# MegviiRobot/CamLaserCalibraTool

Measured on NVIDIA H100. Metric: residual+Jacobian evals/sec (full LM solves), higher is better.
Workload: dtype f64

## Files before the change

camlasercalibratool_b200/_build.py:

```python
from __future__ import annotations

import os
import shutil
import subprocess

PKG_DIR = os.path.dirname(os.path.abspath(__file__))
CSRC = os.path.join(PKG_DIR, "csrc")
LIB_PATH = os.path.join(PKG_DIR, "libclc_b200.so")
SOURCES = ["clc_api.cu", "clc_pack.cpp"]
HEADERS = ["clc_kernels.cuh", "clc_math.cuh", "clc_lm.cuh", "clc_expand.cuh", "clc_linefit.cuh", "clc_camera.cuh", "clc_upload.inl"]
NVCC_FLAGS = [
    "-gencode", "arch=compute_90a,code=sm_90a",
    "-O3", "-lineinfo", "-std=c++17",
    "-shared", "-Xcompiler", "-fPIC",
    "-diag-suppress", "177",
]


def _nvcc() -> str:
    for cand in (shutil.which("nvcc"), "/usr/local/cuda/bin/nvcc"):
        if cand and os.path.exists(cand):
            return cand
    raise RuntimeError("nvcc not found: libclc_b200.so cannot be built")


def is_stale() -> bool:
    if not os.path.exists(LIB_PATH):
        return True
    t = os.path.getmtime(LIB_PATH)
    deps = [os.path.join(CSRC, f) for f in SOURCES + HEADERS]
    deps.append(os.path.join(PKG_DIR, "..", "include", "clc_b200.h"))
    return any(os.path.getmtime(d) > t for d in deps)


def build(force: bool = False, verbose: bool = False) -> str:
    if not force and not is_stale():
        return LIB_PATH
    extra = os.environ.get("CLC_NVCC_EXTRA", "").split()
    out = os.environ.get("CLC_LIB_OUT", LIB_PATH)
    cmd = [_nvcc(), *NVCC_FLAGS, *extra, "-o", out, *[os.path.join(CSRC, s) for s in SOURCES], "-ldl"]
    if verbose:
        cmd.insert(1, "-Xptxas")
        cmd.insert(2, "-v")
    res = subprocess.run(cmd, capture_output=True, text=True)
    if res.returncode != 0:
        raise RuntimeError("nvcc failed:\n" + res.stdout + res.stderr)
    if verbose:
        print(res.stderr)
    return out


REPO = os.path.dirname(PKG_DIR)
DROPIN_SRC = os.path.join(PKG_DIR, "host", "LaseCamCalB200.cpp")
BENCH_SRC = os.path.join(PKG_DIR, "host", "dropin_bench.cpp")
BENCH_EXE = os.path.join(PKG_DIR, "host", "clc_dropin_bench")
def interface_include_dirs():
    return [os.path.join(REPO, "tests", "stubs"), os.path.join(REPO, "include")]


def cxx_command(sources, out, extra=()):
    cxx = "/usr/bin/g++" if os.path.exists("/usr/bin/g++") else "g++"
    cmd = [cxx, "-O2", "-std=c++11", "-Wall"]
    for d in interface_include_dirs():
# ... 19 lines not shown
```

camlasercalibratool_b200/csrc/clc_api.cu:

```cuda
#include <cuda_runtime.h>
#include <dlfcn.h>
#include <nccl.h>

#include <algorithm>
#include <atomic>
#include <chrono>
#include <cstdio>
#include <cstdlib>
#include <cstring>
#include <mutex>
#include <string>
#include <vector>

#include "../../include/clc_b200.h"
#include "clc_kernels.cuh"
#include "clc_linefit.cuh"
#include "clc_small.cuh"

namespace {

thread_local std::string g_last_error;
std::atomic<int64_t> g_launches{0};

int fail(int code, const std::string& msg) {
  g_last_error = msg;
  return code;
}

#define CLC_CUDA(expr)                                                                                   \
  do {                                                                                                   \
    cudaError_t _e = (expr);                                                                             \
    if (_e != cudaSuccess)                                                                               \
      return fail(CLC_ERR_CUDA, std::string(#expr) + ": " + cudaGetErrorString(_e) + " (" __FILE__ ":" + \
                                    std::to_string(__LINE__) + ")");                                     \
  } while (0)

#define CLC_LAUNCH_CHECK()                  \
  do {                                      \
    g_launches.fetch_add(1);                \
    CLC_CUDA(cudaGetLastError());           \
  } while (0)

struct NcclApi {
  void* handle = nullptr;
  ncclResult_t (*GetUniqueId)(ncclUniqueId*) = nullptr;
  ncclResult_t (*CommInitRank)(ncclComm_t*, int, ncclUniqueId, int) = nullptr;
  ncclResult_t (*AllReduce)(const void*, void*, size_t, ncclDataType_t, ncclRedOp_t, ncclComm_t, cudaStream_t) = nullptr;
  ncclResult_t (*CommDestroy)(ncclComm_t) = nullptr;
  const char* (*GetErrorString)(ncclResult_t) = nullptr;
  std::string error;
};

NcclApi* nccl_api() {
  static NcclApi api;
  static bool tried = false;
  if (tried) return &api;
  tried = true;
  const char* names[] = {"libnccl.so.2", "libnccl.so"};
  for (const char* n : names) {
    api.handle = dlopen(n, RTLD_NOW | RTLD_GLOBAL);
    if (api.handle) break;
  }
  if (!api.handle) {
    api.error = std::string("dlopen(libnccl.so.2) failed: ") + dlerror();
    return &api;
  }
  api.GetUniqueId = reinterpret_cast<decltype(api.GetUniqueId)>(dlsym(api.handle, "ncclGetUniqueId"));
  api.CommInitRank = reinterpret_cast<decltype(api.CommInitRank)>(dlsym(api.handle, "ncclCommInitRank"));
// ... 102 lines not shown
  }
  for (int i = 0; i < n; ++i) x[perm[i]] = y[i];
}

int64_t round_up(int64_t v, int64_t m) { return (v + m - 1) / m * m; }

}

struct PinnedBlock {
  clc::LmState lm;
  double sums[clc::kMaxOut];
  double pose[8];
  int done;
  int nonplanar;
};
namespace {
std::mutex g_pinned_mutex;
std::vector<PinnedBlock*> g_pinned_free;
PinnedBlock* pinned_acquire() {
  {
    std::lock_guard<std::mutex> lock(g_pinned_mutex);
    if (!g_pinned_free.empty()) {
      PinnedBlock* b = g_pinned_free.back();
      g_pinned_free.pop_back();
      return b;
    }
  }
  PinnedBlock* b = nullptr;
  if (cudaMallocHost(&b, sizeof(PinnedBlock)) != cudaSuccess) return nullptr;
  return b;
}
void pinned_release(PinnedBlock* b) {
  if (!b) return;
  std::lock_guard<std::mutex> lock(g_pinned_mutex);
  g_pinned_free.push_back(b);
}
}

struct clc_comm {
  ncclComm_t comm = nullptr;
  int nranks = 1, rank = 0, device = 0;
  void* p2p_block = nullptr;
  void* peer_block[clc::kMaxRanks] = {};
  bool p2p_ready = false;
  bool local = false;
  size_t mailbox_bytes() const { return sizeof(unsigned long long) * 2 * 2 * (size_t)nranks * clc::kMailboxSlot; }
  size_t block_bytes() const { return mailbox_bytes() + sizeof(unsigned long long); }
};

struct clc_problem {
  int device = 0;
  cudaStream_t stream = nullptr;
  int num_sms = 0;
  int grid = 0;
  int64_t n_frames = 0, n_points = 0, n_points_padded = 0, n_edges = 0;
  int use_loss = 1;
  double cauchy_a = 0.05;
  double *x = nullptr, *y = nullptr, *z = nullptr;
  void *xy_block = nullptr, *z_block = nullptr;
  double* frame_pose = nullptr;
  double* frame_pose_true = nullptr;
  double* plane = nullptr;
  int64_t* offsets = nullptr;
  int* warp_first_frame = nullptr;
  double* edge_plane = nullptr;
  double* edge_pt = nullptr;
  unsigned long long* partials_ll = nullptr;
  unsigned int* launch_seq = nullptr;
  unsigned long long* pose_ll = nullptr;
  double* sums = nullptr;
  double* pose = nullptr;
  clc::LmState* lm = nullptr;
  double* flush_buf = nullptr;
  int64_t flush_n = 0;
  unsigned long long* timing = nullptr;
  bool use_pdl = true;
  int64_t l2_persist_bytes = 0;
  bool l2_window_set = false;
  bool small_kernel = true;
  int loop_in_kernel = 1;
  PinnedBlock* pinned = nullptr;
  double* h_sums = nullptr;
  int* h_done = nullptr;
  clc::LmState* h_lm = nullptr;
  clc_comm* comm_obj = nullptr;
  ncclComm_t comm = nullptr;
  int nranks = 1, rank = 0;
  int* p2p_error = nullptr;
  int allreduce_mode = 0;
  int64_t per_warp = 0;
  int grid_full = 0;
  cudaEvent_t ev0 = nullptr, ev1 = nullptr;
  int* d_nonplanar = nullptr;
  bool z_all_zero = false;
  bool host_planarity_known = false;
  bool planar = false;
  int planar_mode = 1;
  int64_t planar_min_points = 0;
};

namespace {

clc::ProblemView make_view(const clc_problem* p) {
  clc::ProblemView v;
  v.x = p->x; v.y = p->y; v.z = p->z;
  v.plane = p->plane;
  v.offsets = p->offsets;
  v.warp_first_frame = p->warp_first_frame;
  v.edge_plane = p->edge_plane;
  v.edge_pt = p->edge_pt;
  v.n_frames = p->n_frames;
  v.n_points = p->n_points;
  v.n_edges = p->n_edges;
  v.per_warp = p->per_warp;
  v.a2 = p->cauchy_a * p->cauchy_a;
  v.inv_a2 = 1.0 / v.a2;
  return v;
}

int set_device(const clc_problem* p) {
  CLC_CUDA(cudaSetDevice(p->device));
  return CLC_OK;
}

int launch_sweep(clc_problem* p, int mode, bool loss, bool edges, const double* d_pose, const int* d_done,
                 clc::LmState* d_lm, bool collective = true, bool pdl = false, int loop_sweeps = 1) {
  clc::SweepArgs a;
  a.pose7 = d_pose;
  a.done = d_done;
  a.partials_ll = p->partials_ll;
  a.sums = p->sums;
  a.launch_seq = p->launch_seq;
  a.pose_ll = p->pose_ll;
  a.lm = d_lm;
  a.use_loss = loss ? 1 : 0;
  a.use_edges = edges ? 1 : 0;
  a.loop_sweeps = loop_sweeps;
  a.timing = p->timing;
  a.nranks = 1;
  a.rank = 0;
  a.seq_counter = nullptr;
  a.error = p->p2p_error;
  if (p->nranks > 1 && p->allreduce_mode == 1 && collective) {
    clc_comm* c = p->comm_obj;
    a.nranks = c->nranks;
    a.rank = c->rank;
    a.seq_counter = reinterpret_cast<unsigned long long*>(static_cast<char*>(c->p2p_block) + c->mailbox_bytes());
    for (int r = 0; r < c->nranks; ++r) a.peer_mailbox[r] = static_cast<unsigned long long*>(c->peer_block[r]);
  }
  const clc::ProblemView v = make_view(p);
  cudaLaunchConfig_t cfg = {};
  cfg.gridDim = dim3((unsigned)p->grid);
  cfg.blockDim = dim3(clc::kThreads);
  cfg.dynamicSmemBytes = clc::dyn_smem_bytes(p->planar);
  cfg.stream = p->stream;
  cudaLaunchAttribute attr[1];
  attr[0].id = cudaLaunchAttributeProgrammaticStreamSerialization;
  attr[0].val.programmaticStreamSerializationAllowed = pdl ? 1 : 0;
  cfg.attrs = attr;
  cfg.numAttrs = 1;
  cudaError_t le;
  if (!p->planar && p->z == nullptr) return fail(CLC_ERR_INVALID, "internal: general sweep without a z stream");
  if (mode == clc::kModeClosedForm) {
    le = p->planar ? cudaLaunchKernelEx(&cfg, clc::clc_sweep_kernel<false, clc::kModeClosedForm, true>, v, a)
                   : cudaLaunchKernelEx(&cfg, clc::clc_sweep_kernel<false, clc::kModeClosedForm, false>, v, a);
  } else if (loop_sweeps > 1) {
    if (d_lm == nullptr) return fail(CLC_ERR_INVALID, "internal: looping sweep without an LM state");
    if (loss)
      le = p->planar ? cudaLaunchKernelEx(&cfg, clc::clc_sweep_kernel<true, clc::kModeLM, true, true>, v, a)
                     : cudaLaunchKernelEx(&cfg, clc::clc_sweep_kernel<true, clc::kModeLM, false, true>, v, a);
    else
      le = p->planar ? cudaLaunchKernelEx(&cfg, clc::clc_sweep_kernel<false, clc::kModeLM, true, true>, v, a)
                     : cudaLaunchKernelEx(&cfg, clc::clc_sweep_kernel<false, clc::kModeLM, false, true>, v, a);
  } else if (loss) {
    le = p->planar ? cudaLaunchKernelEx(&cfg, clc::clc_sweep_kernel<true, clc::kModeLM, true>, v, a)
                   : cudaLaunchKernelEx(&cfg, clc::clc_sweep_kernel<true, clc::kModeLM, false>, v, a);
  } else {
    le = p->planar ? cudaLaunchKernelEx(&cfg, clc::clc_sweep_kernel<false, clc::kModeLM, true>, v, a)
                   : cudaLaunchKernelEx(&cfg, clc::clc_sweep_kernel<false, clc::kModeLM, false>, v, a);
  }
  if (le != cudaSuccess) return fail(CLC_ERR_CUDA, std::string("sweep launch: ") + cudaGetErrorString(le));
  CLC_LAUNCH_CHECK();
  return CLC_OK;
}

int allreduce_sums(clc_problem* p, int count) {
  if (p->nranks <= 1 || p->allreduce_mode == 1) return CLC_OK;
  CLC_NCCL(nccl_api()->AllReduce(p->sums, p->sums, (size_t)count, ncclDouble, ncclSum, p->comm, p->stream));
  return CLC_OK;
}

cudaError_t sync_stream_low_latency(cudaStream_t st) {
  const auto t0 = std::chrono::steady_clock::now();
  for (;;) {
    const cudaError_t e = cudaStreamQuery(st);
    if (e != cudaErrorNotReady) return e;
    if (std::chrono::steady_clock::now() - t0 > std::chrono::microseconds(400)) return cudaStreamSynchronize(st);
#if defined(__x86_64__) || defined(__i386__)
    __builtin_ia32_pause();
#endif
  }
}

int check_p2p_error(clc_problem* p) {
  if (p->grid <= 1 && p->nranks <= 1) return CLC_OK;
  int err = 0;
  CLC_CUDA(cudaMemcpyAsync(&err, p->p2p_error, sizeof(int), cudaMemcpyDeviceToHost, p->stream));
  CLC_CUDA(sync_stream_low_latency(p->stream));
  if (err == 2) return fail(CLC_ERR_CUDA, "sweep kernel: the persistent grid was not co-resident (ticket wait timed out)");
  if (err) return fail(CLC_ERR_NCCL, "peer exchange timed out: a rank did not reach the collective");
  return CLC_OK;
}

int materialise_z(clc_problem* p);

int partition(clc_problem* p) {
  const int chunk = p->planar ? clc::kPlanarChunk : clc::kChunk;
  p->grid = p->grid_full;
  {
    const int64_t stages = (p->n_points + chunk - 1) / chunk;
    const int64_t blocks_needed = std::max<int64_t>(1, (stages + clc::kWarps - 1) / clc::kWarps);
    if (blocks_needed < p->grid) p->grid = (int)blocks_needed;
    int64_t single_block_max = (int64_t)clc::kWarps * 8 * clc::kChunk;
    if (const char* env = std::getenv("CLC_SINGLE_BLOCK_MAX_POINTS")) single_block_max = std::atoll(env);
    if (p->n_points <= single_block_max) p->grid = 1;
  }
  const int64_t n_warps = (int64_t)p->grid * clc::kWarps;
  p->per_warp = std::max<int64_t>(chunk, round_up((p->n_points + n_warps - 1) / n_warps, chunk));
  if (p->warp_first_frame) CLC_CUDA(cudaFreeAsync(p->warp_first_frame, p->stream));
  if (p->partials_ll) CLC_CUDA(cudaFreeAsync(p->partials_ll, p->stream));
  p->warp_first_frame = nullptr;
  p->partials_ll = nullptr;
  CLC_CUDA(cudaMallocAsync(&p->warp_first_frame, sizeof(int) * n_warps, p->stream));
  const size_t ll_bytes = sizeof(unsigned long long) * 2 * (size_t)p->grid * clc::kMaxOut;
  CLC_CUDA(cudaMallocAsync(&p->partials_ll, ll_bytes, p->stream));
  CLC_CUDA(cudaMemsetAsync(p->partials_ll, 0, ll_bytes, p->stream));
  const int threads = 256;
  const int blocks = (int)((n_warps + threads - 1) / threads);
  clc::clc_warp_table_kernel<<<blocks, threads, 0, p->stream>>>(p->offsets, p->n_frames, p->n_points, p->per_warp, n_warps,
                                                                p->warp_first_frame);
  CLC_LAUNCH_CHECK();
  return CLC_OK;
}

int finish_create(clc_problem* p) {
  const int threads = 256;
  if (p->n_frames > 0) {
    const int blocks = (int)((p->n_frames + threads - 1) / threads);
    clc::clc_planes_kernel<<<blocks, threads, 0, p->stream>>>(p->frame_pose, p->n_frames, p->plane, p->edge_plane);
    CLC_LAUNCH_CHECK();
  }
  static std::mutex cfg_mutex;
  static int cached_blocks_per_sm[64] = {};
  int blocks_per_sm = 0;
  {
    std::lock_guard<std::mutex> lock(cfg_mutex);
    if (p->device < 64) blocks_per_sm = cached_blocks_per_sm[p->device];
  }
  if (blocks_per_sm == 0) {
    int occ = 0, occ_min = 1 << 30;
    const void* variants[] = {
        (const void*)clc::clc_sweep_kernel<true, clc::kModeLM, false>,         (const void*)clc::clc_sweep_kernel<true, clc::kModeLM, true>,
        (const void*)clc::clc_sweep_kernel<false, clc::kModeLM, false>,        (const void*)clc::clc_sweep_kernel<false, clc::kModeLM, true>,
        (const void*)clc::clc_sweep_kernel<false, clc::kModeClosedForm, false>, (const void*)clc::clc_sweep_kernel<false, clc::kModeClosedForm, true>,
        (const void*)clc::clc_sweep_kernel<true, clc::kModeLM, false, true>,   (const void*)clc::clc_sweep_kernel<true, clc::kModeLM, true, true>,
        (const void*)clc::clc_sweep_kernel<false, clc::kModeLM, false, true>,  (const void*)clc::clc_sweep_kernel<false, clc::kModeLM, true, true>};
    for (int v = 0; v < 10; ++v) {
      const void* fn = variants[v];
      const int smem = clc::dyn_smem_bytes((v & 1) != 0);
      CLC_CUDA(cudaFuncSetAttribute(fn, cudaFuncAttributeMaxDynamicSharedMemorySize, smem));
      CLC_CUDA(cudaOccupancyMaxActiveBlocksPerMultiprocessor(&occ, fn, clc::kThreads, smem));
      occ_min = std::min(occ_min, occ);
    }
    if (occ_min < 1) return fail(CLC_ERR_CUDA, "the sweep kernel does not fit on this device");
    blocks_per_sm = std::max(1, std::min(occ_min, clc::kBlocksPerSM));
    if (const char* env = std::getenv("CLC_BLOCKS_PER_SM")) {
      const int v = std::atoi(env);
      if (v >= 1) blocks_per_sm = std::min(v, std::max(1, occ_min));
    }
    std::lock_guard<std::mutex> lock(cfg_mutex);
    if (p->device < 64) cached_blocks_per_sm[p->device] = blocks_per_sm;
  }
  p->grid_full = p->num_sms * blocks_per_sm;
  if (const char* env = std::getenv("CLC_PDL")) p->use_pdl = std::atoi(env) != 0;
  if (const char* env = std::getenv("CLC_LOOP_IN_KERNEL")) p->loop_in_kernel = std::atoi(env);
  if (const char* env = std::getenv("CLC_SMALL_KERNEL")) p->small_kernel = std::atoi(env) != 0;
  if (const char* env = std::getenv("CLC_L2_PERSIST_MB")) p->l2_persist_bytes = (int64_t)std::atoll(env) << 20;
  CLC_CUDA(cudaMallocAsync(&p->sums, sizeof(double) * clc::kMaxOut, p->stream));
  CLC_CUDA(cudaMallocAsync(&p->pose, sizeof(double) * 8, p->stream));
  CLC_CUDA(cudaMallocAsync(&p->launch_seq, sizeof(unsigned int), p->stream));
  CLC_CUDA(cudaMallocAsync(&p->pose_ll, sizeof(unsigned long long) * 16, p->stream));
  CLC_CUDA(cudaMemsetAsync(p->pose_ll, 0, sizeof(unsigned long long) * 16, p->stream));
  CLC_CUDA(cudaMallocAsync(&p->lm, sizeof(clc::LmState), p->stream));
  CLC_CUDA(cudaMallocAsync(&p->p2p_error, sizeof(int), p->stream));
  CLC_CUDA(cudaMemsetAsync(p->p2p_error, 0, sizeof(int), p->stream));
  CLC_CUDA(cudaMemsetAsync(p->launch_seq, 0, sizeof(unsigned int), p->stream));
  CLC_CUDA(cudaMemsetAsync(p->sums, 0, sizeof(double) * clc::kMaxOut, p->stream));
  p->pinned = pinned_acquire();
  if (!p->pinned) return fail(CLC_ERR_CUDA, "cudaMallocHost failed");
  p->h_sums = p->pinned->sums;
  p->h_done = &p->pinned->done;
  p->h_lm = &p->pinned->lm;
  if (p->host_planarity_known) {
    CLC_CUDA(cudaStreamSynchronize(p->stream));
  } else {
    p->pinned->nonplanar = 1;
    CLC_CUDA(cudaMemcpyAsync(&p->pinned->nonplanar, p->d_nonplanar, sizeof(int), cudaMemcpyDeviceToHost, p->stream));
    CLC_CUDA(cudaStreamSynchronize(p->stream));
    p->z_all_zero = p->pinned->nonplanar == 0;
  }
  if (const char* env = std::getenv("CLC_PLANAR")) p->planar_mode = std::atoi(env) != 0 ? 1 : 0;
  p->planar_min_points = (int64_t)p->grid_full * clc::kWarps * clc::kPlanarChunk;
  if (const char* env = std::getenv("CLC_PLANAR_MIN_POINTS")) p->planar_min_points = std::atoll(env);
  p->planar = p->z_all_zero && p->planar_mode != 0 && p->n_points >= p->planar_min_points;
  if (p->planar && p->z != nullptr) {
    CLC_CUDA(cudaFreeAsync(p->z_block, p->stream));
    p->z = nullptr;
    p->z_block = nullptr;
  } else if (!p->planar) {
    int rc = materialise_z(p);
    if (rc != CLC_OK) return rc;
  }
  return partition(p);
}

int init_device(clc_problem* p, int device) {
  int count = 0;
  CLC_CUDA(cudaGetDeviceCount(&count));
  if (count <= 0) return fail(CLC_ERR_CUDA, "no CUDA device");
  if (device < 0) CLC_CUDA(cudaGetDevice(&device));
  if (device >= count) return fail(CLC_ERR_INVALID, "device ordinal out of range");
  p->device = device;
  CLC_CUDA(cudaSetDevice(device));
  struct DeviceInfo { bool valid = false; int major = 0, minor = 0, sms = 0; };
  static std::mutex info_mutex;
  static DeviceInfo info[64];
  DeviceInfo di;
  {
    std::lock_guard<std::mutex> lock(info_mutex);
    if (device < 64) di = info[device];
  }
  if (!di.valid) {
    CLC_CUDA(cudaDeviceGetAttribute(&di.major, cudaDevAttrComputeCapabilityMajor, device));
    CLC_CUDA(cudaDeviceGetAttribute(&di.minor, cudaDevAttrComputeCapabilityMinor, device));
    CLC_CUDA(cudaDeviceGetAttribute(&di.sms, cudaDevAttrMultiProcessorCount, device));
    cudaMemPool_t pool;
    CLC_CUDA(cudaDeviceGetDefaultMemPool(&pool, device));
    uint64_t threshold = UINT64_MAX;
    CLC_CUDA(cudaMemPoolSetAttribute(pool, cudaMemPoolAttrReleaseThreshold, &threshold));
    di.valid = true;
    std::lock_guard<std::mutex> lock(info_mutex);
    if (device < 64) info[device] = di;
  }
  if (di.major != 9 || di.minor != 0)
    return fail(CLC_ERR_CUDA, std::string("libclc_b200 is built for sm_90a only; device is sm_") + std::to_string(di.major) +
                                  std::to_string(di.minor));
  p->num_sms = di.sms;
  CLC_CUDA(cudaStreamCreateWithFlags(&p->stream, cudaStreamNonBlocking));
  return CLC_OK;
}

int64_t env_skew(const char* name, int64_t dflt) {
  const char* env = std::getenv(name);
  if (!env) return dflt;
  const int64_t v = std::atoll(env);
  return v < 0 ? 0 : (v / 512) * 512;
}
constexpr int64_t kSkewPeriod = (int64_t)2 << 20;

int alloc_z(clc_problem* p) {
  const size_t bytes = sizeof(double) * (size_t)p->n_points_padded;
  CLC_CUDA(cudaMallocAsync(&p->z_block, bytes + (size_t)kSkewPeriod, p->stream));
  const int64_t want = env_skew("CLC_SKEW_Z", 0) % kSkewPeriod;
  const int64_t have = (int64_t)((reinterpret_cast<uintptr_t>(p->z_block) - reinterpret_cast<uintptr_t>(p->x)) % (uintptr_t)kSkewPeriod);
  const int64_t shift = ((want - have) % kSkewPeriod + kSkewPeriod) % kSkewPeriod;
  p->z = reinterpret_cast<double*>(static_cast<char*>(p->z_block) + shift);
  if (std::getenv("CLC_DEBUG_LAYOUT")) std::fprintf(stderr, "CLC_DEBUG_LAYOUT x=%p y=%p z=%p (z block %p)\n", (void*)p->x, (void*)p->y, (void*)p->z, p->z_block);
  return CLC_OK;
}

int alloc_points(clc_problem* p, bool with_z) {
  p->n_points_padded = round_up(p->n_points, clc::kMaxChunk) + clc::kMaxChunk;
  const size_t bytes = sizeof(double) * (size_t)p->n_points_padded;
  const int64_t congruent = (kSkewPeriod - (int64_t)(bytes % (size_t)kSkewPeriod)) % kSkewPeriod;
  const int64_t skew_y = env_skew("CLC_SKEW_Y", bytes >= (size_t)(4 * kSkewPeriod) ? congruent : 0);
  CLC_CUDA(cudaMallocAsync(&p->xy_block, 2 * bytes + (size_t)skew_y, p->stream));
  p->x = static_cast<double*>(p->xy_block);
  p->y = reinterpret_cast<double*>(static_cast<char*>(p->xy_block) + bytes + skew_y);
  if (with_z) {
    int rc = alloc_z(p);
    if (rc != CLC_OK) return rc;
  }
  CLC_CUDA(cudaMallocAsync(&p->d_nonplanar, sizeof(int), p->stream));
  CLC_CUDA(cudaMemsetAsync(p->d_nonplanar, 0, sizeof(int), p->stream));
  const int64_t tail = p->n_points_padded - p->n_points;
  CLC_CUDA(cudaMemsetAsync(p->x + p->n_points, 0, sizeof(double) * tail, p->stream));
  CLC_CUDA(cudaMemsetAsync(p->y + p->n_points, 0, sizeof(double) * tail, p->stream));
  if (with_z) CLC_CUDA(cudaMemsetAsync(p->z + p->n_points, 0, sizeof(double) * tail, p->stream));
  return CLC_OK;
}

int materialise_z(clc_problem* p) {
  if (p->z != nullptr) return CLC_OK;
  int rc = alloc_z(p);
  if (rc != CLC_OK) return rc;
  CLC_CUDA(cudaMemsetAsync(p->z, 0, sizeof(double) * (size_t)p->n_points_padded, p->stream));
  return CLC_OK;
}

}
// ... 510 lines not shown
  if (p->l2_persist_bytes <= 0 || !p->xy_block) return CLC_OK;
  if (on == p->l2_window_set) return CLC_OK;
  cudaStreamAttrValue attr;
  std::memset(&attr, 0, sizeof(attr));
  if (on) {
    int max_persist = 0, max_window = 0;
    CLC_CUDA(cudaDeviceGetAttribute(&max_persist, cudaDevAttrMaxPersistingL2CacheSize, p->device));
    CLC_CUDA(cudaDeviceGetAttribute(&max_window, cudaDevAttrMaxAccessPolicyWindowSize, p->device));
    const size_t set_aside = (size_t)std::min<int64_t>(p->l2_persist_bytes, max_persist);
    if (set_aside == 0 || max_window <= 0) return CLC_OK;
    size_t cur = 0;
    CLC_CUDA(cudaDeviceGetLimit(&cur, cudaLimitPersistingL2CacheSize));
    if (cur < set_aside) CLC_CUDA(cudaDeviceSetLimit(cudaLimitPersistingL2CacheSize, set_aside));
    const size_t span = sizeof(double) * (size_t)(p->y - p->x) + sizeof(double) * (size_t)p->n_points;
    const size_t window = std::min(span, (size_t)max_window);
    attr.accessPolicyWindow.base_ptr = p->xy_block;
    attr.accessPolicyWindow.num_bytes = window;
    attr.accessPolicyWindow.hitRatio = (float)std::min(1.0, (double)set_aside / (double)window);
    attr.accessPolicyWindow.hitProp = cudaAccessPropertyPersisting;
    attr.accessPolicyWindow.missProp = cudaAccessPropertyStreaming;
  } else {
    attr.accessPolicyWindow.num_bytes = 0;
  }
  CLC_CUDA(cudaStreamSetAttribute(p->stream, cudaStreamAttributeAccessPolicyWindow, &attr));
  p->l2_window_set = on;
  return CLC_OK;
}

int solve_begin(clc_problem* p, const double pose7[7], const clc_lm_options& opt, SolveCtx* ctx) {
  int rc = set_device(p);
  if (rc != CLC_OK) return rc;
  rc = l2_window(p, true);
  if (rc != CLC_OK) return rc;
  ctx->opt = opt;
  clc::lm_init(&p->h_lm->core, pose7, opt);
  if (!p->ev0) CLC_CUDA(cudaEventCreate(&p->ev0));
  if (!p->ev1) CLC_CUDA(cudaEventCreate(&p->ev1));
  if (p->p2p_error) CLC_CUDA(cudaMemsetAsync(p->p2p_error, 0, sizeof(int), p->stream));
  CLC_CUDA(cudaMemcpyAsync(&p->lm->core, &p->h_lm->core, sizeof(clc::LmCore), cudaMemcpyHostToDevice, p->stream));
  CLC_CUDA(cudaEventRecord(p->ev0, p->stream));
  ctx->fused_update = (p->nranks <= 1) || p->allreduce_mode == 1;
  ctx->loss = p->use_loss != 0;
  ctx->edges = p->n_edges > 0;
  ctx->max_sweeps = opt.max_num_iterations + 2;
  ctx->launched = 0;
  *p->h_done = 0;
  return CLC_OK;
}

int solve_launch_one(clc_problem* p, SolveCtx* ctx, int loop_sweeps = 1) {
  int rc = set_device(p);
  if (rc != CLC_OK) return rc;
  rc = launch_sweep(p, clc::kModeLM, ctx->loss, ctx->edges, p->lm->core.cand, &p->lm->core.done,
                    ctx->fused_update ? p->lm : nullptr, true, ctx->fused_update && p->use_pdl, loop_sweeps);
  if (rc != CLC_OK) return rc;
  if (!ctx->fused_update) {
    rc = allreduce_sums(p, clc::kNumSums);
    if (rc != CLC_OK) return rc;
    clc::clc_lm_kernel<<<1, 32, 0, p->stream>>>(p->lm, p->sums);
    CLC_LAUNCH_CHECK();
  }
  ctx->launched++;
  return CLC_OK;
}

int solve_poll_enqueue(clc_problem* p) {
  int rc = set_device(p);
  if (rc != CLC_OK) return rc;
  CLC_CUDA(cudaMemcpyAsync(p->h_done, &p->lm->core.done, sizeof(int), cudaMemcpyDeviceToHost, p->stream));
  return CLC_OK;
}

int solve_finish(clc_problem* p, double pose7[7], clc_lm_summary* summary, clc_lm_iteration* trace, int trace_cap) {
  int rc = set_device(p);
  if (rc != CLC_OK) return rc;
  CLC_CUDA(cudaEventRecord(p->ev1, p->stream));
  rc = l2_window(p, false);
  if (rc != CLC_OK) return rc;
  CLC_CUDA(cudaMemcpyAsync(p->h_lm, p->lm, sizeof(clc::LmState), cudaMemcpyDeviceToHost, p->stream));
  CLC_CUDA(sync_stream_low_latency(p->stream));
  float ms = 0.f;
  CLC_CUDA(cudaEventElapsedTime(&ms, p->ev0, p->ev1));
  rc = check_p2p_error(p);
  if (rc != CLC_OK) return rc;
  const clc::LmCore& s = p->h_lm->core;
  const clc_lm_iteration* dev_trace = p->h_lm->trace;
  if (pose7)
    for (int i = 0; i < 7; ++i) pose7[i] = s.x[i];
  if (summary) {
    summary->termination = s.done ? s.done : CLC_TERM_NO_CONVERGENCE;
    summary->num_iterations = s.n_trace;
    summary->num_successful_steps = s.num_successful;
    summary->num_unsuccessful_steps = s.num_unsuccessful;
    summary->num_sweeps = s.sweeps;
    summary->reserved = 0;
    summary->initial_cost = s.initial_cost;
    summary->final_cost = s.x_cost;
    summary->device_ms = ms;
  }
  if (trace) {
    const int n = std::min(std::min(s.n_trace, clc::kTraceMax), trace_cap);
    for (int i = 0; i < n; ++i) trace[i] = dev_trace[i];
  }
  return CLC_OK;
}

int solve_all(clc_problem* const* ps, int n, double pose7[7], const clc_lm_options* opt_in, clc_lm_summary* summary,
              clc_lm_iteration* trace, int trace_cap) {
  clc_lm_options opt;
  if (opt_in) opt = *opt_in; else clc_lm_default_options(&opt);
  if (opt.max_num_iterations < 0) return fail(CLC_ERR_INVALID, "max_num_iterations < 0");
  if (opt.iterations_per_sync < 1) opt.iterations_per_sync = 1;
  std::vector<SolveCtx> ctx((size_t)n);
  int rc = CLC_OK;
  for (int g = 0; g < n && rc == CLC_OK; ++g) rc = solve_begin(ps[g], pose7, opt, &ctx[g]);
  if (rc != CLC_OK) return rc;
  const int max_sweeps = ctx[0].max_sweeps;
  int launched = 0;
  if (n == 1 && ps[0]->small_kernel && ps[0]->loop_in_kernel >= 1 && ps[0]->nranks <= 1 && ctx[0].fused_update &&
      ps[0]->n_points + (ctx[0].edges ? ps[0]->n_edges : 0) <= clc::kSmallMaxResiduals) {
    clc_problem* p = ps[0];
    rc = set_device(p);
    if (rc != CLC_OK) return rc;
    const clc::ProblemView v = make_view(p);
    if (ctx[0].loss)
      clc::clc_small_lm_kernel<true><<<clc::kSmallCluster, clc::kSmallThreads, 0, p->stream>>>(v, p->lm, max_sweeps, ctx[0].edges ? 1 : 0, nullptr, nullptr);
    else
      clc::clc_small_lm_kernel<false><<<clc::kSmallCluster, clc::kSmallThreads, 0, p->stream>>>(v, p->lm, max_sweeps, ctx[0].edges ? 1 : 0, nullptr, nullptr);
    CLC_LAUNCH_CHECK();
    launched = max_sweeps;
  }
  bool loop_launch = launched == 0;
  for (int g = 0; g < n; ++g)
    loop_launch = loop_launch && ctx[g].fused_update &&
                  (ps[g]->loop_in_kernel >= 2 || (ps[g]->loop_in_kernel == 1 && ps[g]->grid == 1 && ps[g]->nranks <= 1));
  if (loop_launch) {
    for (int g = 0; g < n; ++g) {
      rc = solve_launch_one(ps[g], &ctx[g], max_sweeps);
      if (rc != CLC_OK) return rc;
    }
    launched = max_sweeps;
  }
  while (launched < max_sweeps) {
    const int batch = std::min(launched == 0 ? 2 * opt.iterations_per_sync : opt.iterations_per_sync, max_sweeps - launched);
    for (int i = 0; i < batch; ++i)
      for (int g = 0; g < n; ++g) {
        rc = solve_launch_one(ps[g], &ctx[g]);
        if (rc != CLC_OK) return rc;
      }
    launched += batch;
    for (int g = 0; g < n; ++g) {
      rc = solve_poll_enqueue(ps[g]);
      if (rc != CLC_OK) return rc;
    }
    bool all_done = true;
    for (int g = 0; g < n; ++g) {
      rc = set_device(ps[g]);
      if (rc != CLC_OK) return rc;
      CLC_CUDA(sync_stream_low_latency(ps[g]->stream));
      all_done = all_done && (*ps[g]->h_done != 0);
    }
    if (all_done) break;
  }
  double ms_max = 0.0;
  int first_rc = CLC_OK;
  for (int g = n - 1; g >= 0; --g) {
    clc_lm_summary sg;
    rc = solve_finish(ps[g], g == 0 ? pose7 : nullptr, &sg, g == 0 ? trace : nullptr, trace_cap);
    if (rc != CLC_OK && first_rc == CLC_OK) first_rc = rc;
    if (rc == CLC_OK) {
      ms_max = std::max(ms_max, sg.device_ms);
      if (g == 0 && summary) *summary = sg;
    }
  }
  if (first_rc != CLC_OK) return first_rc;
  if (summary) summary->device_ms = ms_max;
  return CLC_OK;
}

}

int clc_solve_lm(clc_problem* p, double pose7[7], const clc_lm_options* opt_in, clc_lm_summary* summary,
                 clc_lm_iteration* trace, int trace_cap) {
  if (!p || !pose7) return fail(CLC_ERR_INVALID, "NULL argument");
  return solve_all(&p, 1, pose7, opt_in, summary, trace, trace_cap);
}


int clc_problem_line_fit(clc_problem* p, double* lines, int max_num_iterations, double* info) {
  if (!p || !lines || max_num_iterations < 0) return fail(CLC_ERR_INVALID, "bad line-fit arguments");
  int rc = set_device(p);
  if (rc != CLC_OK) return rc;
  const int64_t N = p->n_frames;
  if (N == 0) return CLC_OK;
  double *d_lines = nullptr, *d_info = nullptr;
  cudaError_t e = cudaMallocAsync(&d_lines, sizeof(double) * 2 * N, p->stream);
  if (e == cudaSuccess && info) e = cudaMallocAsync(&d_info, sizeof(double) * 4 * N, p->stream);
  if (e == cudaSuccess) e = cudaMemcpyAsync(d_lines, lines, sizeof(double) * 2 * N, cudaMemcpyHostToDevice, p->stream);
  if (e == cudaSuccess) {
    const int warps = 8;
    clc::clc_line_fit_kernel<<<(unsigned)((N + warps - 1) / warps), warps * 32, 0, p->stream>>>(
        p->x, p->y, p->offsets, N, max_num_iterations, p->cauchy_a, d_lines, d_info);
    g_launches.fetch_add(1);
    e = cudaGetLastError();
  }
  if (e == cudaSuccess) e = cudaMemcpyAsync(lines, d_lines, sizeof(double) * 2 * N, cudaMemcpyDeviceToHost, p->stream);
  if (e == cudaSuccess && info) e = cudaMemcpyAsync(info, d_info, sizeof(double) * 4 * N, cudaMemcpyDeviceToHost, p->stream);
  if (e == cudaSuccess) e = cudaStreamSynchronize(p->stream);
  if (d_lines) cudaFreeAsync(d_lines, p->stream);
  if (d_info) cudaFreeAsync(d_info, p->stream);
  if (e != cudaSuccess) return fail(CLC_ERR_CUDA, cudaGetErrorString(e));
  return CLC_OK;
}

namespace {
struct LineFitCache {
// ... 745 lines not shown
```

camlasercalibratool_b200/csrc/clc_kernels.cuh:

```cuda
#pragma once

#include <cuda_runtime.h>

#include "clc_camera.cuh"
#include "clc_expand.cuh"
#include "clc_lm.cuh"

namespace clc {

#ifndef CLC_THREADS
#define CLC_THREADS 384
#endif
#ifndef CLC_BLOCKS_PER_SM
#define CLC_BLOCKS_PER_SM 1
#endif
#ifndef CLC_STAGES
#define CLC_STAGES 2
#endif
constexpr int kThreads = CLC_THREADS;
constexpr int kBlocksPerSM = CLC_BLOCKS_PER_SM;
constexpr int kWarps = kThreads / 32;
constexpr int kTileStride = 13;
#ifndef CLC_CHUNK
#define CLC_CHUNK 128
#endif
constexpr int kChunk = CLC_CHUNK;
constexpr int kGroups = kChunk / 64;
constexpr int kStages = CLC_STAGES;
constexpr int kMaxOut = 54;
constexpr int kMaxRanks = 16;
constexpr int kMailboxSlot = 64;
#ifndef CLC_PLANAR_STAGES
#define CLC_PLANAR_STAGES CLC_STAGES
#endif
#ifndef CLC_PLANAR_CHUNK
#define CLC_PLANAR_CHUNK (CLC_CHUNK * 2)
#endif
constexpr int kPlanarStages = CLC_PLANAR_STAGES;
constexpr int kPlanarChunk = CLC_PLANAR_CHUNK;
static_assert(kChunk % 64 == 0 && kPlanarChunk % 64 == 0, "stages are made of 64-point groups");
constexpr int kMaxChunk = kChunk > kPlanarChunk ? kChunk : kPlanarChunk;
#ifndef CLC_LOCKSTEP_SLACK
#define CLC_LOCKSTEP_SLACK 0
#endif
constexpr int kLockstepSlack = CLC_LOCKSTEP_SLACK;
constexpr int kBarsPerWarp = kStages > kPlanarStages ? kStages : kPlanarStages;
constexpr int kTileDoublesPerWarp = 32 * kTileStride;
__host__ __device__ constexpr int ring_doubles_per_warp(bool planar) { return planar ? kPlanarStages * 2 * kPlanarChunk : kStages * 3 * kChunk; }
__host__ __device__ constexpr int dyn_smem_bytes(bool planar) {
  return kWarps * ring_doubles_per_warp(planar) * 8 + kWarps * kTileDoublesPerWarp * 8 + kWarps * kBarsPerWarp * 8;
}

enum SweepMode { kModeLM = 0, kModeClosedForm = 1 };

struct ProblemView {
  const double* x;
  const double* y;
  const double* z;
  const double* plane;
  const int64_t* offsets;
  const int* warp_first_frame;
  const double* edge_plane;
  const double* edge_pt;
  int64_t n_frames;
  int64_t n_points;
  int64_t n_edges;
  int64_t per_warp;
  double inv_a2;
  double a2;
};

struct SweepArgs {
  const double* pose7;
  const int* done;
  unsigned long long* partials_ll;
  double* sums;
  unsigned int* launch_seq;
  LmState* lm;
  int use_loss;
  int use_edges;
  int loop_sweeps;
  unsigned long long* pose_ll;
  unsigned long long* timing;
  int nranks;
  int rank;
  unsigned long long* seq_counter;
  unsigned long long* peer_mailbox[kMaxRanks];
  int* error;
};


__device__ __forceinline__ unsigned long long globaltimer_ns() {
  unsigned long long t;
  asm volatile("mov.u64 %0, %globaltimer;" : "=l"(t));
  return t;
}
#define CLC_STAMP(slot)                                                                       \
  do {                                                                                        \
    if (args.timing != nullptr && threadIdx.x == 0) args.timing[(int64_t)blockIdx.x * 8 + (slot)] = globaltimer_ns(); \
  } while (0)

__device__ __forceinline__ uint32_t smem_u32(const void* p) { return (uint32_t)__cvta_generic_to_shared(p); }

__device__ __forceinline__ void mbar_init(uint64_t* bar, uint32_t count) {
  asm volatile("mbarrier.init.shared::cta.b64 [%0], %1;" ::"r"(smem_u32(bar)), "r"(count) : "memory");
}
__device__ __forceinline__ void mbar_expect_tx(uint64_t* bar, uint32_t bytes) {
  asm volatile("mbarrier.arrive.expect_tx.shared::cta.b64 _, [%0], %1;" ::"r"(smem_u32(bar)), "r"(bytes) : "memory");
}
__device__ __forceinline__ void mbar_wait(uint64_t* bar, uint32_t parity) {
  uint32_t done;
  do {
    asm volatile(
        "{\n\t.reg .pred p;\n\t"
        "mbarrier.try_wait.parity.shared::cta.b64 p, [%1], %2;\n\t"
        "selp.u32 %0, 1, 0, p;\n\t}"
        : "=r"(done)
        : "r"(smem_u32(bar)), "r"(parity)
        : "memory");
  } while (!done);
}
__device__ __forceinline__ void bulk_g2s(void* dst, const void* src, uint32_t bytes, uint64_t* bar) {
  asm volatile("cp.async.bulk.shared::cluster.global.mbarrier::complete_tx::bytes [%0], [%1], %2, [%3];" ::"r"(
                   smem_u32(dst)),
               "l"(src), "r"(bytes), "r"(smem_u32(bar))
               : "memory");
}

__device__ __forceinline__ void st_relaxed_sys(unsigned long long* p, unsigned long long v) {
  asm volatile("st.relaxed.sys.global.u64 [%0], %1;" ::"l"(p), "l"(v) : "memory");
}
__device__ __forceinline__ unsigned long long ld_relaxed_sys(const unsigned long long* p) {
  unsigned long long v;
  asm volatile("ld.relaxed.sys.global.u64 %0, [%1];" : "=l"(v) : "l"(p) : "memory");
  return v;
}

__device__ __forceinline__ void st_volatile_v2(unsigned long long* p, unsigned long long a, unsigned long long b) {
  asm volatile("st.volatile.global.v2.u64 [%0], {%1, %2};" ::"l"(p), "l"(a), "l"(b) : "memory");
}
__device__ __forceinline__ void ld_volatile_v2(const unsigned long long* p, unsigned long long& a, unsigned long long& b) {
  asm volatile("ld.volatile.global.v2.u64 {%0, %1}, [%2];" : "=l"(a), "=l"(b) : "l"(p) : "memory");
}

__device__ __forceinline__ unsigned int ld_acquire_gpu(const unsigned int* p) {
  unsigned int v;
  asm volatile("ld.acquire.gpu.global.u32 %0, [%1];" : "=r"(v) : "l"(p) : "memory");
  return v;
}
__device__ __forceinline__ unsigned int atom_add_acq_rel_gpu(unsigned int* p, unsigned int v) {
  unsigned int old;
  asm volatile("atom.acq_rel.gpu.global.add.u32 %0, [%1], %2;" : "=r"(old) : "l"(p), "r"(v) : "memory");
  return old;
}

__device__ __forceinline__ double rcp_pos(double a) {
  double r;
  asm("rcp.approx.ftz.f64 %0, %1;" : "=d"(r) : "d"(a));
  double e = fma(-a, r, 1.0);
  r = fma(r, e, r);
  e = fma(-a, r, 1.0);
  r = fma(r, e, r);
  return r;
}

__device__ __forceinline__ double warp_sum(double v) {
#pragma unroll
  for (int o = 16; o > 0; o >>= 1) v += __shfl_xor_sync(0xffffffffu, v, o);
  return v;
}

template <int N>
__device__ __forceinline__ void warp_transpose_sum(double* v, int lane) {
#pragma unroll
  for (int half = N / 2; half >= 1; half >>= 1) {
    const bool upper = (lane & half) != 0;
#pragma unroll
    for (int i = 0; i < half; ++i) {
      const double keep = upper ? v[i + half] : v[i];
// ... 58 lines not shown
    accumulate<PLANAR>(a, v0 ? 1.0 : 0.0, X.x, Y.x, Z.x);
    accumulate<PLANAR>(a, v1 ? 1.0 : 0.0, X.y, Y.y, Z.y);
  }
}

__device__ __forceinline__ void renormalise(Moments& a) {
  const int hi = __double2hiint(a.prod);
  const int ex = (hi >> 20) - 1023;
  a.esum += ex;
  a.prod = __hiloint2double(hi - (ex << 20), __double2loint(a.prod));
}

template <bool LOSS, int MODE, bool PLANAR, bool LOOP = false>
__global__ void __launch_bounds__(kThreads, kBlocksPerSM)
clc_sweep_kernel(ProblemView pv, SweepArgs args) {
  constexpr int NOUT = (MODE == kModeLM) ? kNumSums : kMaxOut;
  constexpr int NST = PLANAR ? kPlanarStages : kStages;
  constexpr int CH = PLANAR ? kPlanarChunk : kChunk;
  constexpr int G = CH / 64;
  constexpr int SST = (PLANAR ? 2 : 3) * CH;
  constexpr int RING = NST * SST;
  static_assert(RING == ring_doubles_per_warp(PLANAR), "ring size");
  extern __shared__ __align__(128) unsigned char s_dyn[];
  __shared__ double s_acc[kWarps][NOUT];
  __shared__ double s_red[kWarps][32];
  __shared__ unsigned long long s_core[kLmCoreWords];
  __shared__ double s_next[8];
  __shared__ int s_prog[32];

  CLC_STAMP(0);
  if (args.timing != nullptr && threadIdx.x == 0) {
    unsigned int smid;
    asm volatile("mov.u32 %0, %smid;" : "=r"(smid));
    args.timing[(int64_t)blockIdx.x * 8 + 7] = smid;
  }

  const int lane = threadIdx.x & 31;
  const int warp = threadIdx.x >> 5;
  const int64_t gwarp = (int64_t)blockIdx.x * kWarps + warp;

  const int64_t P = pv.n_points;
  int64_t p0 = gwarp * pv.per_warp;
  if (p0 > P) p0 = P;
  int64_t p1 = p0 + pv.per_warp;
  if (p1 > P) p1 = P;
  const int n_chunks = (int)((p1 - p0 + CH - 1) / CH);
  double* ring = reinterpret_cast<double*>(s_dyn) + warp * RING;
  double* tile = reinterpret_cast<double*>(s_dyn) + kWarps * RING + warp * kTileDoublesPerWarp;
  uint64_t* bars = reinterpret_cast<uint64_t*>(s_dyn + (size_t)kWarps * (RING + kTileDoublesPerWarp) * 8) + warp * kBarsPerWarp;

  const int sweeps_max = (LOOP && args.loop_sweeps > 1 && MODE == kModeLM && args.lm != nullptr) ? args.loop_sweeps : 1;
  const int total_chunks = LOOP ? sweeps_max * n_chunks : n_chunks;
  int issued = 0, next_c = 0;
  auto issue_one = [&](bool slot_was_read) {
    if (lane == 0) {
      const int c = LOOP ? next_c : issued, st = issued % NST;
      double* dst = ring + st * SST;
      const int64_t src = p0 + (int64_t)c * CH;
      if (slot_was_read) asm volatile("fence.proxy.async.shared::cta;" ::: "memory");
      mbar_expect_tx(bars + st, (PLANAR ? 2 : 3) * CH * 8);
      bulk_g2s(dst, pv.x + src, CH * 8, bars + st);
      bulk_g2s(dst + CH, pv.y + src, CH * 8, bars + st);
      if (!PLANAR) bulk_g2s(dst + 2 * CH, pv.z + src, CH * 8, bars + st);
    }
    ++issued;
    if (LOOP && ++next_c == n_chunks) next_c = 0;
  };
  auto drain = [&](int g) {
    for (; g < issued; ++g) mbar_wait(bars + g % NST, (uint32_t)(g / NST) & 1u);
  };
  if (lane == 0) {
#pragma unroll
    for (int st = 0; st < NST; ++st) mbar_init(bars + st, 1);
    asm volatile("fence.mbarrier_init.release.cluster;" ::: "memory");
    asm volatile("fence.proxy.async.shared::cta;" ::: "memory");
  }
  __syncwarp();
  for (int g = 0; g < NST && g < total_chunks; ++g) issue_one(false);
  __syncwarp();

  asm volatile("griddepcontrol.wait;" ::: "memory");
  if (args.done != nullptr && (*args.done != 0 || (args.error != nullptr && *args.error != 0))) {
    drain(0);
    return;
  }

  const unsigned int launch_tag0 = *args.launch_seq + 1u;
  if (MODE == kModeLM && args.lm != nullptr && blockIdx.x == 0) {
    const unsigned long long* g_core = reinterpret_cast<const unsigned long long*>(&args.lm->core);
    for (int k = threadIdx.x; k < kLmCoreWords; k += kThreads) s_core[k] = __ldcg(g_core + k);
  }

  PoseConsts pc;
  int n_tile = 0;

  auto flush_tile = [&]() {
    double out[NOUT];
#pragma unroll
    for (int k = 0; k < NOUT; ++k) out[k] = 0.0;
    __syncwarp();
    if (lane < n_tile) {
      const double* row = tile + lane * kTileStride;
      const int64_t f = __double_as_longlong(row[12]);
      double plane[4];
#pragma unroll
      for (int k = 0; k < 4; ++k) plane[k] = pv.plane[f * 4 + k];
      if (MODE == kModeLM) {
        double m[3], c;
        frame_consts(pc, plane, m, &c);
        const double cnt = (double)(pv.offsets[f + 1] - pv.offsets[f]);
        double cost_term = row[10];
        if (LOSS) cost_term = log(row[10]) + row[11] * 0.693147180559945309417232121458;
        expand_lm(plane, m, c, 1.0 / cnt, row, LOSS, cost_term, pv.a2, out);
      } else {
        expand_closed_form(plane, row, out);
      }
// ... 455 lines not shown
    if (ok) ok = camera_estimate_pose(cam, seed, frame_begin + i, fp, fe, uv);
    if (!ok)
      for (int k = 0; k < 7; ++k) fe[k] = fp[k];
  }
  for (int k = 0; k < 7; ++k) {
    frame_pose[i * 7 + k] = fe[k];
    if (frame_pose_true != nullptr) frame_pose_true[i * 7 + k] = fp[k];
  }
  offsets[i] = i * beams;
  if (with_edges) {
    double ep[6];
    if (!gen_edge_points(fp, ep))
      for (int k = 0; k < 6; ++k) ep[k] = 0.0;
    for (int k = 0; k < 6; ++k) edge_pt[i * 6 + k] = ep[k];
  }
}

__global__ void clc_gen_points_kernel(uint64_t seed, double sigma, int64_t frame_begin, int64_t beams,
                                      const double* __restrict__ frame_pose, double* __restrict__ x,
                                      double* __restrict__ y, double* __restrict__ z) {
  const int64_t i = blockIdx.x;
  __shared__ double s_nl[3], s_dl, s_a, s_b;
  if (threadIdx.x == 0) {
    double fp[7], nl[3], dl, a = 0.0, b = 0.0;
    for (int k = 0; k < 7; ++k) fp[k] = frame_pose[i * 7 + k];
    gen_plane_laser(fp, nl, &dl);
    gen_window(nl, dl, &a, &b);
    s_nl[0] = nl[0]; s_nl[1] = nl[1]; s_nl[2] = nl[2]; s_dl = dl; s_a = a; s_b = b;
  }
  __syncthreads();
  const double n0 = s_nl[0], n1 = s_nl[1], dl = s_dl, a = s_a, b = s_b;
  for (int64_t j = threadIdx.x; j < beams; j += blockDim.x) {
    const double theta = a + (b - a) * (((double)j + 0.5) / (double)beams);
    const double cx = cos(theta), sy = sin(theta);
    const double depth = -dl / (cx * n0 + sy * n1) + gen_noise(seed, sigma, frame_begin + i, j);
    const int64_t o = i * beams + j;
    x[o] = depth * cx;
    y[o] = depth * sy;
    if (z != nullptr) z[o] = 0.0;
  }
}

__global__ void clc_flush_kernel(double* buf, int64_t n, double v) {
  for (int64_t i = (int64_t)blockIdx.x * blockDim.x + threadIdx.x; i < n; i += (int64_t)gridDim.x * blockDim.x)
    buf[i] = v;
}
__global__ void clc_flush_read_kernel(const double* buf, int64_t n, double* sink) {
  double acc = 0.0;
  for (int64_t i = (int64_t)blockIdx.x * blockDim.x + threadIdx.x; i < n; i += (int64_t)gridDim.x * blockDim.x)
    acc += __ldcg(buf + i);
  if (acc == 123.456) *sink = acc;
}

}
```

Before: 86.51 billion.

## Pin tail chunks of point stream in L2 with evict_last cache hints

Computes a per-warp count of trailing chunks that fit in half of L2 and issues bulk copies for those chunks with an evict_last policy, while all other chunks use evict_first. Across repeated LM sweeps, the data reloaded each sweep should then come partly from L2 instead of HBM. A demote kernel resets the priority to evict_normal when a solve finishes. This adds policy creation on every copy and an extra kernel per solve, and the hints are disabled for small, latency-bound problems or when a persistence window is already set.

```diff
diff --git a/camlasercalibratool_b200/_build.py b/camlasercalibratool_b200/_build.py
--- a/camlasercalibratool_b200/_build.py
+++ b/camlasercalibratool_b200/_build.py
@@ -8,7 +8,7 @@
 CSRC = os.path.join(PKG_DIR, "csrc")
 LIB_PATH = os.path.join(PKG_DIR, "libclc_b200.so")
 SOURCES = ["clc_api.cu", "clc_pack.cpp"]
-HEADERS = ["clc_kernels.cuh", "clc_math.cuh", "clc_lm.cuh", "clc_expand.cuh", "clc_linefit.cuh", "clc_camera.cuh", "clc_upload.inl"]
+HEADERS = ["clc_kernels.cuh", "clc_math.cuh", "clc_lm.cuh", "clc_expand.cuh", "clc_linefit.cuh", "clc_camera.cuh", "clc_upload.inl", "clc_l2_plan.h"]
 NVCC_FLAGS = [
     "-gencode", "arch=compute_90a,code=sm_90a",
     "-O3", "-lineinfo", "-std=c++17",
diff --git a/camlasercalibratool_b200/csrc/clc_api.cu b/camlasercalibratool_b200/csrc/clc_api.cu
--- a/camlasercalibratool_b200/csrc/clc_api.cu
+++ b/camlasercalibratool_b200/csrc/clc_api.cu
@@ -14,6 +14,7 @@
 
 #include "../../include/clc_b200.h"
 #include "clc_kernels.cuh"
+#include "clc_l2_plan.h"
 #include "clc_linefit.cuh"
 #include "clc_small.cuh"
 
@@ -222,6 +223,7 @@
   int device = 0;
   cudaStream_t stream = nullptr;
   int num_sms = 0;
+  int64_t l2_bytes = 0;
   int grid = 0;
   int64_t n_frames = 0, n_points = 0, n_points_padded = 0, n_edges = 0;
   int use_loss = 1;
@@ -247,6 +249,8 @@
   bool use_pdl = true;
   int64_t l2_persist_bytes = 0;
   bool l2_window_set = false;
+  int64_t l2_resident_bytes = -1;
+  int resident_chunks = 0;
   bool small_kernel = true;
   int loop_in_kernel = 1;
   PinnedBlock* pinned = nullptr;
@@ -283,6 +287,7 @@
   v.n_points = p->n_points;
   v.n_edges = p->n_edges;
   v.per_warp = p->per_warp;
+  v.resident_chunks = p->resident_chunks;
   v.a2 = p->cauchy_a * p->cauchy_a;
   v.inv_a2 = 1.0 / v.a2;
   return v;
@@ -294,7 +299,7 @@
 }
 
 int launch_sweep(clc_problem* p, int mode, bool loss, bool edges, const double* d_pose, const int* d_done,
-                 clc::LmState* d_lm, bool collective = true, bool pdl = false, int loop_sweeps = 1) {
+                 clc::LmState* d_lm, bool collective = true, bool pdl = false, int loop_sweeps = 1, bool l2_hints = false) {
   clc::SweepArgs a;
   a.pose7 = d_pose;
   a.done = d_done;
@@ -305,6 +310,7 @@
   a.lm = d_lm;
   a.use_loss = loss ? 1 : 0;
   a.use_edges = edges ? 1 : 0;
+  a.l2_hints = l2_hints ? 1 : 0;
   a.loop_sweeps = loop_sweeps;
   a.timing = p->timing;
   a.nranks = 1;
@@ -404,6 +410,12 @@
   CLC_CUDA(cudaMallocAsync(&p->warp_first_frame, sizeof(int) * n_warps, p->stream));
   const size_t ll_bytes = sizeof(unsigned long long) * 2 * (size_t)p->grid * clc::kMaxOut;
   CLC_CUDA(cudaMallocAsync(&p->partials_ll, ll_bytes, p->stream));
+  {
+    const int64_t stage_bytes = (int64_t)(p->planar ? 2 : 3) * chunk * 8;
+    const bool latency_bound = p->n_points <= clc::kSmallMaxResiduals;
+    const int64_t budget = p->l2_persist_bytes > 0 ? 0 : clc::l2_resident_budget(p->l2_bytes, p->l2_resident_bytes);
+    p->resident_chunks = clc::l2_resident_chunks(budget, p->grid, clc::kWarps, p->per_warp / chunk, stage_bytes, latency_bound);
+  }
   CLC_CUDA(cudaMemsetAsync(p->partials_ll, 0, ll_bytes, p->stream));
   const int threads = 256;
   const int blocks = (int)((n_warps + threads - 1) / threads);
@@ -456,6 +468,7 @@
   if (const char* env = std::getenv("CLC_LOOP_IN_KERNEL")) p->loop_in_kernel = std::atoi(env);
   if (const char* env = std::getenv("CLC_SMALL_KERNEL")) p->small_kernel = std::atoi(env) != 0;
   if (const char* env = std::getenv("CLC_L2_PERSIST_MB")) p->l2_persist_bytes = (int64_t)std::atoll(env) << 20;
+  if (const char* env = std::getenv("CLC_L2_RESIDENT_MB")) p->l2_resident_bytes = std::max<int64_t>(0, (int64_t)std::atoll(env) << 20);
   CLC_CUDA(cudaMallocAsync(&p->sums, sizeof(double) * clc::kMaxOut, p->stream));
   CLC_CUDA(cudaMallocAsync(&p->pose, sizeof(double) * 8, p->stream));
   CLC_CUDA(cudaMallocAsync(&p->launch_seq, sizeof(unsigned int), p->stream));
@@ -502,7 +515,7 @@
   if (device >= count) return fail(CLC_ERR_INVALID, "device ordinal out of range");
   p->device = device;
   CLC_CUDA(cudaSetDevice(device));
-  struct DeviceInfo { bool valid = false; int major = 0, minor = 0, sms = 0; };
+  struct DeviceInfo { bool valid = false; int major = 0, minor = 0, sms = 0, l2 = 0; };
   static std::mutex info_mutex;
   static DeviceInfo info[64];
   DeviceInfo di;
@@ -514,6 +527,7 @@
     CLC_CUDA(cudaDeviceGetAttribute(&di.major, cudaDevAttrComputeCapabilityMajor, device));
     CLC_CUDA(cudaDeviceGetAttribute(&di.minor, cudaDevAttrComputeCapabilityMinor, device));
     CLC_CUDA(cudaDeviceGetAttribute(&di.sms, cudaDevAttrMultiProcessorCount, device));
+    CLC_CUDA(cudaDeviceGetAttribute(&di.l2, cudaDevAttrL2CacheSize, device));
     cudaMemPool_t pool;
     CLC_CUDA(cudaDeviceGetDefaultMemPool(&pool, device));
     uint64_t threshold = UINT64_MAX;
@@ -526,6 +540,7 @@
     return fail(CLC_ERR_CUDA, std::string("libclc_b200 is built for sm_90a only; device is sm_") + std::to_string(di.major) +
                                   std::to_string(di.minor));
   p->num_sms = di.sms;
+  p->l2_bytes = di.l2;
   CLC_CUDA(cudaStreamCreateWithFlags(&p->stream, cudaStreamNonBlocking));
   return CLC_OK;
 }
@@ -1142,7 +1157,8 @@
   int rc = set_device(p);
   if (rc != CLC_OK) return rc;
   rc = launch_sweep(p, clc::kModeLM, ctx->loss, ctx->edges, p->lm->core.cand, &p->lm->core.done,
-                    ctx->fused_update ? p->lm : nullptr, true, ctx->fused_update && p->use_pdl, loop_sweeps);
+                    ctx->fused_update ? p->lm : nullptr, true, ctx->fused_update && p->use_pdl, loop_sweeps,
+                    true);
   if (rc != CLC_OK) return rc;
   if (!ctx->fused_update) {
     rc = allreduce_sums(p, clc::kNumSums);
@@ -1161,8 +1177,21 @@
   return CLC_OK;
 }
 
+int l2_demote(clc_problem* p) {
+  if (p->resident_chunks == 0) return CLC_OK;
+  int rc = set_device(p);
+  if (rc != CLC_OK) return rc;
+  const int chunk = p->planar ? clc::kPlanarChunk : clc::kChunk;
+  const int64_t n_warps = (int64_t)p->grid * clc::kWarps;
+  const int64_t lines = n_warps * p->resident_chunks * (chunk / 16);
+  const int threads = 256;
+  clc::clc_l2_demote_kernel<<<(unsigned)((lines + threads - 1) / threads), threads, 0, p->stream>>>(make_view(p), n_warps, chunk);
+  CLC_LAUNCH_CHECK();
+  return CLC_OK;
+}
+
 int solve_finish(clc_problem* p, double pose7[7], clc_lm_summary* summary, clc_lm_iteration* trace, int trace_cap) {
-  int rc = set_device(p);
+  int rc = l2_demote(p);
   if (rc != CLC_OK) return rc;
   CLC_CUDA(cudaEventRecord(p->ev1, p->stream));
   rc = l2_window(p, false);
@@ -1205,6 +1234,15 @@
   int rc = CLC_OK;
   for (int g = 0; g < n && rc == CLC_OK; ++g) rc = solve_begin(ps[g], pose7, opt, &ctx[g]);
   if (rc != CLC_OK) return rc;
+  struct DemoteOnExit {
+    clc_problem* const* ps;
+    int n;
+    bool armed;
+    ~DemoteOnExit() {
+      if (armed)
+        for (int g = 0; g < n; ++g) l2_demote(ps[g]);
+    }
+  } demote_on_exit{ps, n, true};
   const int max_sweeps = ctx[0].max_sweeps;
   int launched = 0;
   if (n == 1 && ps[0]->small_kernel && ps[0]->loop_in_kernel >= 1 && ps[0]->nranks <= 1 && ctx[0].fused_update &&
@@ -1252,6 +1290,7 @@
     }
     if (all_done) break;
   }
+  demote_on_exit.armed = false;
   double ms_max = 0.0;
   int first_rc = CLC_OK;
   for (int g = n - 1; g >= 0; --g) {
diff --git a/camlasercalibratool_b200/csrc/clc_kernels.cuh b/camlasercalibratool_b200/csrc/clc_kernels.cuh
--- a/camlasercalibratool_b200/csrc/clc_kernels.cuh
+++ b/camlasercalibratool_b200/csrc/clc_kernels.cuh
@@ -66,6 +66,7 @@
   int64_t n_points;
   int64_t n_edges;
   int64_t per_warp;
+  int resident_chunks;
   double inv_a2;
   double a2;
 };
@@ -79,6 +80,7 @@
   LmState* lm;
   int use_loss;
   int use_edges;
+  int l2_hints;
   int loop_sweeps;
   unsigned long long* pose_ll;
   unsigned long long* timing;
@@ -125,6 +127,22 @@
                    smem_u32(dst)),
                "l"(src), "r"(bytes), "r"(smem_u32(bar))
                : "memory");
+}
+__device__ __forceinline__ void bulk_g2s_hint(void* dst, const void* src, uint32_t bytes, uint64_t* bar, uint64_t policy) {
+  asm volatile("cp.async.bulk.shared::cluster.global.mbarrier::complete_tx::bytes.L2::cache_hint [%0], [%1], %2, [%3], %4;" ::"r"(
+                   smem_u32(dst)),
+               "l"(src), "r"(bytes), "r"(smem_u32(bar)), "l"(policy)
+               : "memory");
+}
+__device__ __forceinline__ uint64_t policy_evict_last() {
+  uint64_t pol;
+  asm("createpolicy.fractional.L2::evict_last.b64 %0, 1.0;" : "=l"(pol));
+  return pol;
+}
+__device__ __forceinline__ uint64_t policy_evict_first() {
+  uint64_t pol;
+  asm("createpolicy.fractional.L2::evict_first.b64 %0, 1.0;" : "=l"(pol));
+  return pol;
 }
 
 __device__ __forceinline__ void st_relaxed_sys(unsigned long long* p, unsigned long long v) {
@@ -289,6 +307,7 @@
   const int sweeps_max = (LOOP && args.loop_sweeps > 1 && MODE == kModeLM && args.lm != nullptr) ? args.loop_sweeps : 1;
   const int total_chunks = LOOP ? sweeps_max * n_chunks : n_chunks;
   int issued = 0, next_c = 0;
+  const bool l2_hints = args.l2_hints != 0 && pv.resident_chunks > 0;
   auto issue_one = [&](bool slot_was_read) {
     if (lane == 0) {
       const int c = LOOP ? next_c : issued, st = issued % NST;
@@ -296,9 +315,16 @@
       const int64_t src = p0 + (int64_t)c * CH;
       if (slot_was_read) asm volatile("fence.proxy.async.shared::cta;" ::: "memory");
       mbar_expect_tx(bars + st, (PLANAR ? 2 : 3) * CH * 8);
-      bulk_g2s(dst, pv.x + src, CH * 8, bars + st);
-      bulk_g2s(dst + CH, pv.y + src, CH * 8, bars + st);
-      if (!PLANAR) bulk_g2s(dst + 2 * CH, pv.z + src, CH * 8, bars + st);
+      if (l2_hints) {
+        const uint64_t pol = c >= n_chunks - pv.resident_chunks ? policy_evict_last() : policy_evict_first();
+        bulk_g2s_hint(dst, pv.x + src, CH * 8, bars + st, pol);
+        bulk_g2s_hint(dst + CH, pv.y + src, CH * 8, bars + st, pol);
+        if (!PLANAR) bulk_g2s_hint(dst + 2 * CH, pv.z + src, CH * 8, bars + st, pol);
+      } else {
+        bulk_g2s(dst, pv.x + src, CH * 8, bars + st);
+        bulk_g2s(dst + CH, pv.y + src, CH * 8, bars + st);
+        if (!PLANAR) bulk_g2s(dst + 2 * CH, pv.z + src, CH * 8, bars + st);
+      }
     }
     ++issued;
     if (LOOP && ++next_c == n_chunks) next_c = 0;
@@ -860,4 +886,24 @@
   if (acc == 123.456) *sink = acc;
 }
 
-}
+__global__ void clc_l2_demote_kernel(ProblemView pv, int64_t n_warps, int chunk) {
+  const int k = pv.resident_chunks;
+  const int64_t lines_per_warp = (int64_t)k * chunk / 16;
+  const int64_t t = (int64_t)blockIdx.x * blockDim.x + threadIdx.x;
+  if (t >= n_warps * lines_per_warp) return;
+  const int64_t w = t / lines_per_warp;
+  const int64_t P = pv.n_points;
+  int64_t p0 = w * pv.per_warp;
+  if (p0 > P) p0 = P;
+  int64_t p1 = p0 + pv.per_warp;
+  if (p1 > P) p1 = P;
+  const int64_t n_chunks = (p1 - p0 + chunk - 1) / chunk;
+  const int64_t c0 = n_chunks > k ? n_chunks - k : 0;
+  const int64_t i = p0 + c0 * chunk + (t - w * lines_per_warp) * 16;
+  if (i >= p0 + n_chunks * chunk) return;
+  asm volatile("applypriority.global.L2::evict_normal [%0], 128;" ::"l"(pv.x + i) : "memory");
+  asm volatile("applypriority.global.L2::evict_normal [%0], 128;" ::"l"(pv.y + i) : "memory");
+  if (pv.z != nullptr) asm volatile("applypriority.global.L2::evict_normal [%0], 128;" ::"l"(pv.z + i) : "memory");
+}
+
+}
diff --git a/camlasercalibratool_b200/csrc/clc_l2_plan.h b/camlasercalibratool_b200/csrc/clc_l2_plan.h
--- /dev/null
+++ b/camlasercalibratool_b200/csrc/clc_l2_plan.h
@@ -0,0 +1,20 @@
+#pragma once
+
+#include <algorithm>
+#include <cstdint>
+
+namespace clc {
+
+constexpr double kL2ResidentFraction = 0.5;
+
+inline int64_t l2_resident_budget(int64_t l2_bytes, int64_t override_bytes) {
+  return override_bytes >= 0 ? override_bytes : (int64_t)((double)l2_bytes * kL2ResidentFraction);
+}
+
+inline int l2_resident_chunks(int64_t budget_bytes, int64_t grid, int64_t warps_per_block, int64_t stages_per_warp,
+                              int64_t stage_bytes, bool latency_bound) {
+  if (budget_bytes <= 0 || grid <= 1 || latency_bound || stages_per_warp <= 0 || stage_bytes <= 0) return 0;
+  return (int)std::min<int64_t>(stages_per_warp, budget_bytes / (grid * warps_per_block * stage_bytes));
+}
+
+}
```

Measured after the change: 91.07 billion (median of 6 runs). 5.3% higher.
